# BDMstudio/audio-cut

Hardware: AMD Instinct MI355X
Metric: audio-seconds processed/sec (separate+detect) per GPU; cut-point index parity (higher is better)
Workload: dtype f32

## Files before the change

### audio_cut_amd/csrc/ac_tdf_small.hip

```cpp
#include "ac_common.h"

typedef __attribute__((ext_vector_type(4))) float f32x4;

#define TS_ROWS 32
#define TS_HMAX 48
#define TS_HSTRIDE 50
#define TS_OSTRIDE 36

template <int NT1>
__global__ __launch_bounds__(256) void k_tdf_small(const float* __restrict__ x, const float4* __restrict__ w1p,
                                                   const float* __restrict__ w2p, const float* __restrict__ s1,
                                                   const float* __restrict__ b1, const float* __restrict__ s2,
                                                   const float* __restrict__ b2, float* __restrict__ y, long long M, int F,
                                                   int Hd, int T, int C, float* __restrict__ out_amax) {
    __shared__ __attribute__((aligned(16))) float s_h[4][TS_ROWS * TS_HSTRIDE];
    const int lane = threadIdx.x & 63, wave = threadIdx.x >> 6;
    const int r = lane & 15, g = lane >> 4;
    const long long m0 = ((long long)blockIdx.x * 4 + wave) * TS_ROWS;
    if (m0 >= M) return;
    const int n_kk = F / 16;
    const int n_ks2 = (Hd + 3) / 4;
    float* sh = s_h[wave];

    f32x4 acc1[2][NT1];
#pragma unroll
    for (int mt = 0; mt < 2; ++mt)
#pragma unroll
        for (int nt = 0; nt < NT1; ++nt) acc1[mt][nt] = (f32x4){0.f, 0.f, 0.f, 0.f};
    const float* xa0 = x + (m0 + r) * (long long)F + 4 * g;
    const float* xa1 = xa0 + 16LL * F;
    for (int kk = 0; kk < n_kk; ++kk) {
        const float4 a0 = *reinterpret_cast<const float4*>(xa0 + 16 * kk);
        const float4 a1 = *reinterpret_cast<const float4*>(xa1 + 16 * kk);
#pragma unroll
        for (int nt = 0; nt < NT1; ++nt) {
            const float4 b = w1p[((size_t)nt * n_kk + kk) * 64 + lane];
            acc1[0][nt] = __builtin_amdgcn_mfma_f32_16x16x4f32(a0.x, b.x, acc1[0][nt], 0, 0, 0);
            acc1[1][nt] = __builtin_amdgcn_mfma_f32_16x16x4f32(a1.x, b.x, acc1[1][nt], 0, 0, 0);
            acc1[0][nt] = __builtin_amdgcn_mfma_f32_16x16x4f32(a0.y, b.y, acc1[0][nt], 0, 0, 0);
            acc1[1][nt] = __builtin_amdgcn_mfma_f32_16x16x4f32(a1.y, b.y, acc1[1][nt], 0, 0, 0);
            acc1[0][nt] = __builtin_amdgcn_mfma_f32_16x16x4f32(a0.z, b.z, acc1[0][nt], 0, 0, 0);
            acc1[1][nt] = __builtin_amdgcn_mfma_f32_16x16x4f32(a1.z, b.z, acc1[1][nt], 0, 0, 0);
            acc1[0][nt] = __builtin_amdgcn_mfma_f32_16x16x4f32(a0.w, b.w, acc1[0][nt], 0, 0, 0);
            acc1[1][nt] = __builtin_amdgcn_mfma_f32_16x16x4f32(a1.w, b.w, acc1[1][nt], 0, 0, 0);
        }
    }
#pragma unroll
    for (int mt = 0; mt < 2; ++mt) {
#pragma unroll
        for (int i = 0; i < 4; ++i) {
            const int row = mt * 16 + 4 * g + i;
            const int c = (int)(((m0 + row) / T) % C);
            const float sc = s1[c], sf = b1[c];
#pragma unroll
            for (int nt = 0; nt < NT1; ++nt) {
                const int j = nt * 16 + r;
                sh[row * TS_HSTRIDE + j] = (j < Hd) ? fmaxf(acc1[mt][nt][i] * sc + sf, 0.f) : 0.f;
            }
        }
    }
    __builtin_amdgcn_wave_barrier();
    float ha[2][TS_HMAX / 4];
#pragma unroll
    for (int ks = 0; ks < TS_HMAX / 4; ++ks) {
        const int k = 4 * ks + g;
        ha[0][ks] = (ks < n_ks2) ? sh[r * TS_HSTRIDE + k] : 0.f;
        ha[1][ks] = (ks < n_ks2) ? sh[(16 + r) * TS_HSTRIDE + k] : 0.f;
    }
    int crow[2][4];
    float sc2[2][4], sf2[2][4];
#pragma unroll
    for (int mt = 0; mt < 2; ++mt)
#pragma unroll
        for (int i = 0; i < 4; ++i) {
            const int row = mt * 16 + 4 * g + i;
            crow[mt][i] = row;
            const int c = (int)(((m0 + row) / T) % C);
            sc2[mt][i] = s2[c]; sf2[mt][i] = b2[c];
        }
    __builtin_amdgcn_wave_barrier();
    float* so = sh;
    float vmax[4] = {0.f, 0.f, 0.f, 0.f};
    const int orow = lane >> 3, oc4 = lane & 7;
    const int n_nt2 = F / 16;
    for (int nt = 0; nt < n_nt2; nt += 2) {
#pragma unroll
        for (int t = 0; t < 2; ++t) {
            f32x4 acc[2] = {(f32x4){0.f, 0.f, 0.f, 0.f}, (f32x4){0.f, 0.f, 0.f, 0.f}};
            const float* wb = w2p + ((size_t)(nt + t) * n_ks2) * 64 + lane;
#pragma unroll
            for (int ks = 0; ks < TS_HMAX / 4; ++ks) {
                if (ks < n_ks2) {
                    const float b = wb[ks * 64];
                    acc[0] = __builtin_amdgcn_mfma_f32_16x16x4f32(ha[0][ks], b, acc[0], 0, 0, 0);
                    acc[1] = __builtin_amdgcn_mfma_f32_16x16x4f32(ha[1][ks], b, acc[1], 0, 0, 0);
                }
            }
#pragma unroll
            for (int mt = 0; mt < 2; ++mt)
#pragma unroll
                for (int i = 0; i < 4; ++i)
                    so[crow[mt][i] * TS_OSTRIDE + t * 16 + r] = fmaxf(acc[mt][i] * sc2[mt][i] + sf2[mt][i], 0.f);
        }
        __builtin_amdgcn_wave_barrier();
#pragma unroll
        for (int p = 0; p < 4; ++p) {
            const int row = orow + 8 * p;
            const size_t o = (size_t)(m0 + row) * F + nt * 16 + 4 * oc4;
            const float4 t4 = *reinterpret_cast<const float4*>(&so[row * TS_OSTRIDE + 4 * oc4]);
            float4 v = *reinterpret_cast<const float4*>(x + o);
            v.x += t4.x; v.y += t4.y; v.z += t4.z; v.w += t4.w;
            vmax[p] = fmaxf(fmaxf(vmax[p], fmaxf(fabsf(v.x), fabsf(v.y))), fmaxf(fabsf(v.z), fabsf(v.w)));
            *reinterpret_cast<float4*>(y + o) = v;
        }
        __builtin_amdgcn_wave_barrier();
    }
    if (out_amax) {
        float* slots = out_amax + (m0 / ((long long)C * T)) * T;
#pragma unroll
        for (int p = 0; p < 4; ++p) {
            float v = vmax[p];
#pragma unroll
            for (int off = 4; off > 0; off >>= 1) v = fmaxf(v, __shfl_xor(v, off, AC_WAVE));
            if (oc4 == 0 && v > 0.f)
                atomicMax(reinterpret_cast<unsigned*>(slots + (int)((m0 + orow + 8 * p) % T)), __float_as_uint(v));
        }
    }
}

extern "C" int ac_tdf_small_fused(ac_ctx* ctx, const float* x, const void* w1_packed, const void* w2_packed, const float* scale1,
                                  const float* shift1, const float* scale2, const float* shift2, float* y, long long M, int F,
                                  int Hd, int T, int C, float* out_amax, void* stream) {
    AC_REQUIRE(ctx && x && w1_packed && w2_packed && scale1 && shift1 && scale2 && shift2 && y, "null pointer");
    AC_REQUIRE(M > 0 && M % TS_ROWS == 0, "M % 32 == 0");
    AC_REQUIRE(F > 0 && F % 32 == 0, "F % 32 == 0 (the epilogue walks pairs of 16-column tiles)");
    AC_REQUIRE(Hd > 0 && Hd <= TS_HMAX, "bottleneck width in [1, 48]");
    AC_REQUIRE(T > 0 && C > 0, "T, C > 0");
    AC_REQUIRE(!out_amax || ((long long)C * T) % TS_ROWS == 0, "amax needs (C * T) % 32 == 0 (a wave's 32 rows inside one item)");
    AC_REQUIRE(x != y, "in-place not supported (the residual is re-read)");
    const long long n_wave = M / TS_ROWS;
    const long long nblk = (n_wave + 3) / 4;
    AC_REQUIRE(nblk < (1LL << 31), "grid too large");
    dim3 grid((unsigned)nblk), block(256);
    hipStream_t st = (hipStream_t)stream;
    const float4* w1 = (const float4*)w1_packed;
    const float* w2 = (const float*)w2_packed;
    const int nt1 = (Hd + 15) / 16;
    if (nt1 == 3)      hipLaunchKernelGGL(k_tdf_small<3>, grid, block, 0, st, x, w1, w2, scale1, shift1, scale2, shift2, y, M, F, Hd, T, C, out_amax);
    else if (nt1 == 2) hipLaunchKernelGGL(k_tdf_small<2>, grid, block, 0, st, x, w1, w2, scale1, shift1, scale2, shift2, y, M, F, Hd, T, C, out_amax);
    else               hipLaunchKernelGGL(k_tdf_small<1>, grid, block, 0, st, x, w1, w2, scale1, shift1, scale2, shift2, y, M, F, Hd, T, C, out_amax);
    AC_LAUNCH_CHECK();
    return AC_OK;
}
```

Before: 1552.

## Stage x tiles through LDS with coalesced loads and prefetch weights in GEMM1

The first GEMM previously loaded x rows directly in the MFMA fragment layout, where each lane read a float4 from a different row, so loads were poorly coalesced. Now each wave reads 32x32 tiles of x with row-contiguous float4 loads, writes them to its LDS slice and re-reads them in MFMA layout. The next tile and the next packed weight fragments are prefetched one step ahead in registers. This adds LDS traffic, wave barriers and register pressure. It also assumes F is a multiple of 32, which the existing precondition already enforces.

```diff
diff --git a/audio_cut_amd/csrc/ac_tdf_small.hip b/audio_cut_amd/csrc/ac_tdf_small.hip
--- a/audio_cut_amd/csrc/ac_tdf_small.hip
+++ b/audio_cut_amd/csrc/ac_tdf_small.hip
@@ -5,6 +5,7 @@
 #define TS_ROWS 32
 #define TS_HMAX 48
 #define TS_HSTRIDE 50
+#define TS_XSTRIDE 40
 #define TS_OSTRIDE 36
 
 template <int NT1>
@@ -19,6 +20,7 @@
     const long long m0 = ((long long)blockIdx.x * 4 + wave) * TS_ROWS;
     if (m0 >= M) return;
     const int n_kk = F / 16;
+    const int n_kp = n_kk / 2;
     const int n_ks2 = (Hd + 3) / 4;
     float* sh = s_h[wave];
 
@@ -27,24 +29,52 @@
     for (int mt = 0; mt < 2; ++mt)
 #pragma unroll
         for (int nt = 0; nt < NT1; ++nt) acc1[mt][nt] = (f32x4){0.f, 0.f, 0.f, 0.f};
-    const float* xa0 = x + (m0 + r) * (long long)F + 4 * g;
-    const float* xa1 = xa0 + 16LL * F;
-    for (int kk = 0; kk < n_kk; ++kk) {
-        const float4 a0 = *reinterpret_cast<const float4*>(xa0 + 16 * kk);
-        const float4 a1 = *reinterpret_cast<const float4*>(xa1 + 16 * kk);
+    const int lrow = lane >> 3, lc4 = lane & 7;
+    const float* xg = x + (m0 + lrow) * (long long)F + 4 * lc4;
+    f32x4 nx[4];
 #pragma unroll
-        for (int nt = 0; nt < NT1; ++nt) {
-            const float4 b = w1p[((size_t)nt * n_kk + kk) * 64 + lane];
-            acc1[0][nt] = __builtin_amdgcn_mfma_f32_16x16x4f32(a0.x, b.x, acc1[0][nt], 0, 0, 0);
-            acc1[1][nt] = __builtin_amdgcn_mfma_f32_16x16x4f32(a1.x, b.x, acc1[1][nt], 0, 0, 0);
-            acc1[0][nt] = __builtin_amdgcn_mfma_f32_16x16x4f32(a0.y, b.y, acc1[0][nt], 0, 0, 0);
-            acc1[1][nt] = __builtin_amdgcn_mfma_f32_16x16x4f32(a1.y, b.y, acc1[1][nt], 0, 0, 0);
-            acc1[0][nt] = __builtin_amdgcn_mfma_f32_16x16x4f32(a0.z, b.z, acc1[0][nt], 0, 0, 0);
-            acc1[1][nt] = __builtin_amdgcn_mfma_f32_16x16x4f32(a1.z, b.z, acc1[1][nt], 0, 0, 0);
-            acc1[0][nt] = __builtin_amdgcn_mfma_f32_16x16x4f32(a0.w, b.w, acc1[0][nt], 0, 0, 0);
-            acc1[1][nt] = __builtin_amdgcn_mfma_f32_16x16x4f32(a1.w, b.w, acc1[1][nt], 0, 0, 0);
+    for (int p = 0; p < 4; ++p) nx[p] = *reinterpret_cast<const f32x4*>(xg + (long long)(8 * p) * F);
+    f32x4 bc[NT1];
+    const f32x4* w1v = reinterpret_cast<const f32x4*>(w1p);
+#pragma unroll
+    for (int nt = 0; nt < NT1; ++nt) bc[nt] = w1v[((size_t)nt * n_kk) * 64 + lane];
+    for (int kp = 0; kp < n_kp; ++kp) {
+        const int kpn = kp + 1 < n_kp ? kp + 1 : kp;
+#pragma unroll
+        for (int p = 0; p < 4; ++p) *reinterpret_cast<f32x4*>(&sh[(lrow + 8 * p) * TS_XSTRIDE + 4 * lc4]) = nx[p];
+#pragma unroll
+        for (int p = 0; p < 4; ++p) nx[p] = *reinterpret_cast<const f32x4*>(xg + (long long)(8 * p) * F + 32 * kpn);
+        __builtin_amdgcn_wave_barrier();
+        f32x4 a[2][2];
+#pragma unroll
+        for (int h = 0; h < 2; ++h)
+#pragma unroll
+            for (int mt = 0; mt < 2; ++mt) a[h][mt] = *reinterpret_cast<const f32x4*>(&sh[(mt * 16 + r) * TS_XSTRIDE + 16 * h + 4 * g]);
+        __builtin_amdgcn_wave_barrier();
+#pragma unroll
+        for (int h = 0; h < 2; ++h) {
+            const f32x4 a0 = a[h][0], a1 = a[h][1];
+            const int kn = 2 * kp + h + 1;
+            f32x4 bn[NT1];
+#pragma unroll
+            for (int nt = 0; nt < NT1; ++nt) bn[nt] = w1v[((size_t)nt * n_kk + (kn < n_kk ? kn : kn - 1)) * 64 + lane];
+#pragma unroll
+            for (int nt = 0; nt < NT1; ++nt) {
+                const f32x4 b = bc[nt];
+                acc1[0][nt] = __builtin_amdgcn_mfma_f32_16x16x4f32(a0.x, b.x, acc1[0][nt], 0, 0, 0);
+                acc1[1][nt] = __builtin_amdgcn_mfma_f32_16x16x4f32(a1.x, b.x, acc1[1][nt], 0, 0, 0);
+                acc1[0][nt] = __builtin_amdgcn_mfma_f32_16x16x4f32(a0.y, b.y, acc1[0][nt], 0, 0, 0);
+                acc1[1][nt] = __builtin_amdgcn_mfma_f32_16x16x4f32(a1.y, b.y, acc1[1][nt], 0, 0, 0);
+                acc1[0][nt] = __builtin_amdgcn_mfma_f32_16x16x4f32(a0.z, b.z, acc1[0][nt], 0, 0, 0);
+                acc1[1][nt] = __builtin_amdgcn_mfma_f32_16x16x4f32(a1.z, b.z, acc1[1][nt], 0, 0, 0);
+                acc1[0][nt] = __builtin_amdgcn_mfma_f32_16x16x4f32(a0.w, b.w, acc1[0][nt], 0, 0, 0);
+                acc1[1][nt] = __builtin_amdgcn_mfma_f32_16x16x4f32(a1.w, b.w, acc1[1][nt], 0, 0, 0);
+            }
+#pragma unroll
+            for (int nt = 0; nt < NT1; ++nt) bc[nt] = bn[nt];
         }
     }
+    __builtin_amdgcn_wave_barrier();
 #pragma unroll
     for (int mt = 0; mt < 2; ++mt) {
 #pragma unroll
```

Result: no change. 1555, median of 3 (+0.2%).
